# realtimeradio/caltech-bifrost-dsp

Measured on AMD Instinct MI355X. Metric: xengine_ingest_gbps_704in_96ch, higher is better.
Workload: dtype int8 (4+4-bit samples) -> int32

## Files before the change

caltech-bifrost-dsp_amd/csrc/xcorr.hip:

```cpp
#include <algorithm>
#include <cstdlib>
#include <map>
#include <mutex>
#include <vector>

#include "xcorr_kernels.h"
#include "slab.h"
#include "xeng_common.h"

namespace xeng {

struct XgpuConfig {
    int nstand = 352, npol = 2, nchan = 96, ntime_gulp = 480, max_gulps = 0;
};

struct XgpuContext {
    bool live = false;
    int gpu = 0;
    XgpuConfig cfg;
    int ncu = 256;
    int ninput = 0, nblk64 = 0, gkt = 0, cap_kt = 0, cap_gulps = 0, kt_stage = 1;
    int ct_pitch = 0;
    bool raw = false;
    bool kloop16 = false;
    FragGroup* fgroups_dev = nullptr;
    int nfg = 0;
    WorkList work;
    WorkList work_pairs;
    size_t gulp_bytes = 0;
    const uint8_t* gulp_ptr[XC_MAX_GULPS] = {};
    int64_t per_chan = 0, matlen = 0;
    uint8_t* stash[2] = {nullptr, nullptr};
    size_t stash_bytes = 0;
    int cur = 0;
    WgDesc* descs_dev = nullptr;
    int nwg = 0;
    hipStream_t stream = nullptr;
    static constexpr int NMM = 8;
    hipStream_t stream_mm2[NMM] = {};
    int nmm = 2;
    unsigned long long nlaunch = 0;
    hipStream_t stream_mm = nullptr;
    struct Writer { unsigned long long seq; int stream; };
    std::map<const void*, Writer> writers;
    static constexpr int NEV = 256;
    hipEvent_t ev_ring[NEV] = {};
    const void* ring_buf[NEV][2] = {};
    unsigned long long last_seq[NMM] = {};
    hipEvent_t ev_ct = nullptr;
    unsigned long long staging_seen = ~0ull;
    unsigned long long area_seq[2] = {0, 0};
    unsigned long long dump_seq[4] = {0, 0, 0, 0};
    unsigned long long ndump = 0;
    int nfilled = 0;
    bool acc_started = false;
    void* acc_out = nullptr;
    uint8_t* in_dev = nullptr;
    int32_t* out_dev = nullptr;
    unsigned long long* stamps = nullptr;
    GulpDesc* gdesc_dev[2] = {nullptr, nullptr};
    SlabArgs* gargs_dev[2] = {nullptr, nullptr};
    SlabSite slab_site;
    SlabIndexSite slab_index;
    SlabIndexJob slab_job;
    int slab_forced = 0;
    int slab_hint_seen = 0;
    int slab_recent_irr[8] = {}, slab_recent_n[8] = {}, slab_recent_pos = 0;
    unsigned long long slab_tables_until = 0;
    int slab_force_tables = -1;
    bool slab_mode = false;
    EventTimer timer;
};

static std::mutex g_mu;
static XgpuConfig g_cfg;
static XgpuContext g_ctx;
static unsigned long long g_epoch = 1;
// ... 264 lines not shown
    XgpuContext& x = g_ctx;
    if (!x.live || !buf) return 0;
    auto it = x.writers.find(buf);
    return it == x.writers.end() ? 0 : it->second.seq;
}

int xgpu_launches_poll(unsigned long long upto, unsigned long long ctx, bool* done, hipEvent_t* ev, bool exact) {
    std::lock_guard<std::mutex> lk(g_mu);
    XgpuContext& x = g_ctx;
    *done = true;
    if (ev) *ev = nullptr;
    if (upto == 0 || !x.live || ctx != g_ctx_gen) return XENG_STATUS_SUCCESS;
    for (int k = 0; k < (exact ? 1 : x.nmm) && (unsigned long long)k < upto; k++) {
        if (hipEvent_t e = launch_event(upto - k)) {
            const hipError_t q = hipEventQuery(e);
            if (q == hipErrorNotReady) {
                (void)hipGetLastError();
                *done = false;
                if (ev && !*ev) *ev = e;
            } else if (q != hipSuccess) {
                XENG_HIP(q);
            }
        }
    }
    return XENG_STATUS_SUCCESS;
}

int xgpu_pending_poll(unsigned long long seq, unsigned long long epoch, bool* done, bool* launched, hipEvent_t* ev, int* gpu) {
    std::lock_guard<std::mutex> lk(g_mu);
    XgpuContext& x = g_ctx;
    *done = true;
    *launched = true;
    if (ev) *ev = nullptr;
    if (seq == 0 || !x.live || epoch != g_epoch) return XENG_STATUS_SUCCESS;
    if (x.nlaunch < seq) {
        *done = false;
        *launched = false;
        return XENG_STATUS_SUCCESS;
    }
    if (hipEvent_t e = launch_event(seq)) {
        const hipError_t q = hipEventQuery(e);
        if (q == hipErrorNotReady) {
            (void)hipGetLastError();
            *done = false;
            if (ev) *ev = e;
            if (gpu) *gpu = x.gpu;
        } else if (q != hipSuccess) {
            XENG_HIP(q);
        }
    }
    return XENG_STATUS_SUCCESS;
}

}

using namespace xeng;

extern "C" {

int xengXgpuConfigure(int nstand, int npol, int nchan, int ntime_gulp, int max_gulps_per_flush) {
    if (npol != 2) XENG_FAIL(XENG_STATUS_UNSUPPORTED, "xgpu: npol must be 2 (got %d)", npol);
    if (nstand <= 0 || nstand % 4) XENG_FAIL(XENG_STATUS_INVALID_ARGUMENT, "xgpu: nstand must be a positive multiple of 4 (got %d)", nstand);
    if (nstand * npol > 255 * 64) XENG_FAIL(XENG_STATUS_UNSUPPORTED, "xgpu: too many inputs (%d)", nstand * npol);
    if (nchan <= 0 || ntime_gulp <= 0 || max_gulps_per_flush < 0)
        XENG_FAIL(XENG_STATUS_INVALID_ARGUMENT, "xgpu: bad sizes nchan=%d ntime_gulp=%d max_gulps=%d", nchan, ntime_gulp, max_gulps_per_flush);
    std::lock_guard<std::mutex> lk(g_mu);
    g_cfg.nstand = nstand; g_cfg.npol = npol; g_cfg.nchan = nchan; g_cfg.ntime_gulp = ntime_gulp;
    g_cfg.max_gulps = max_gulps_per_flush;
    return XENG_STATUS_SUCCESS;
}

static int initialize_locked(int gpu);

int xengXgpuInitialize(int gpu) {
    std::lock_guard<std::mutex> lk(g_mu);
    destroy_locked();
    const int rc = initialize_locked(gpu);
    if (rc) destroy_locked();
    return rc;
}

static int initialize_locked(int gpu) {
    XgpuContext& x = g_ctx;
    x.cfg = g_cfg;
    x.gpu = gpu < 0 ? 0 : gpu;
    XENG_HIP(hipSetDevice(x.gpu));
    {
        int ncu = 0;
        XENG_HIP(hipDeviceGetAttribute(&ncu, hipDeviceAttributeMultiprocessorCount, x.gpu));
        const char* e = diag_env("XENG_GRID");
        x.ncu = e ? atoi(e) : ncu;
        if (x.ncu < 1) x.ncu = 1;
    }
    x.ninput = x.cfg.nstand * x.cfg.npol;
    x.nblk64 = (x.ninput + 63) / 64;
    x.gkt = (x.cfg.ntime_gulp + 31) / 32;
    x.kt_stage = XC_KT;
    int cap = x.cfg.max_gulps > 0 ? x.cfg.max_gulps : std::max(1, 4800 / (x.gkt * 32));
    cap = std::min(cap, std::max(1, 65535 / (x.gkt * 32)));
    {
        const char* r = getenv("XENG_RAW");
        x.gulp_bytes = (size_t)x.cfg.ntime_gulp * x.cfg.nchan * x.ninput;
        x.raw = !(r && !strcmp(r, "0")) && x.ninput % 16 == 0 &&
                x.cfg.ntime_gulp % (XC_KT * 32) == 0 && x.gulp_bytes + (size_t)16 * x.cfg.nchan * x.ninput < (1ull << 32) &&
                (size_t)x.cfg.nchan * x.ninput >= 128;
        if (x.raw) cap = std::min(cap, XC_MAX_GULPS);
        const char* kl = getenv("XENG_KLOOP");
        x.kloop16 = x.raw && kl && !strcmp(kl, "16");
        const char* st = getenv("XENG_SLAB_TABLES");
        x.slab_force_tables = st ? (strcmp(st, "0") ? 1 : 0) : -1;
        x.slab_hint_seen = 0; x.slab_recent_pos = 0; x.slab_tables_until = 0;
        for (int k = 0; k < 8; k++) x.slab_recent_irr[k] = x.slab_recent_n[k] = 0;
    }
    x.cap_gulps = cap;
    x.cap_kt = ((cap * x.gkt + x.kt_stage - 1) / x.kt_stage) * x.kt_stage;
    x.per_chan = (int64_t)(x.cfg.nstand / 2 + 1) * (x.cfg.nstand / 4) * x.cfg.npol * x.cfg.npol * 4;
    x.matlen = x.per_chan * x.cfg.nchan;
    x.stash_bytes = (size_t)x.cfg.nchan * x.nblk64 * x.cap_kt * KT_BYTES;
    if (x.ninput % 16 == 0) {
        int pitch = x.ninput;
        while (((pitch / 4) & 63) != 8) pitch += 16;
        if ((size_t)16 * pitch + 1024 <= 64 * 1024) x.ct_pitch = pitch;
    }
    if (x.raw) x.stash_bytes = (size_t)cap * x.gulp_bytes;

    for (int b = 0; b < 2; b++) {
        XENG_HIP(hipMalloc((void**)&x.stash[b], x.stash_bytes));
        XENG_HIP(hip_memset_now(x.stash[b], 0, x.stash_bytes));
    }
    XENG_HIP(hipEventCreateWithFlags(&x.ev_ct, hipEventDisableTiming));
    if (x.raw) {
        for (int b = 0; b < 2; b++) {
            XENG_HIP(hipMalloc((void**)&x.gdesc_dev[b], XC_MAX_GULPS * sizeof(GulpDesc)));
            XENG_HIP(hip_memset_now(x.gdesc_dev[b], 0, XC_MAX_GULPS * sizeof(GulpDesc)));
            XENG_HIP(hipMalloc((void**)&x.gargs_dev[b], XC_MAX_GULPS * sizeof(SlabArgs)));
            XENG_HIP(hip_memset_now(x.gargs_dev[b], 0, XC_MAX_GULPS * sizeof(SlabArgs)));
        }
        if (int rcs = slab_site_create(&x.slab_site)) return rcs;
    }
    std::vector<WgDesc> descs = build_wg_descs(x.nblk64);
    x.nwg = (int)descs.size();
    if (x.raw) {
        const bool tiles64 = getenv("XENG_TILING") && !strcmp(getenv("XENG_TILING"), "64");
        const bool plain_order = diag_env("XENG_ITEM_ORDER") && !strcmp(diag_env("XENG_ITEM_ORDER"), "plain");
        const std::vector<FragGroup> groups = tiles64 ? frag_groups_from_tiles(x.nblk64) : build_frag_groups(x.nblk64);
        if (check_frag_groups(groups, x.nblk64) != -1) XENG_FAIL(XENG_STATUS_DEVICE_ERROR, "xgpu: the tiling of %d blocks is not an exact cover", x.nblk64);
        x.nfg = (int)groups.size();
        XENG_HIP(hipMalloc((void**)&x.fgroups_dev, groups.size() * sizeof(FragGroup)));
        XENG_HIP(hipMemcpy(x.fgroups_dev, groups.data(), groups.size() * sizeof(FragGroup), hipMemcpyHostToDevice));
        const std::vector<uint64_t> masks = group_block_masks(groups);
        x.work = build_work(fused_grid(x.cfg.nchan, x.nfg, x.ncu), x.cfg.nchan, x.nfg, plain_order ? nullptr : &masks);
        XENG_HIP(hipMalloc((void**)&x.work.dev, x.work.entries.size() * sizeof(WorkEntry)));
        XENG_HIP(hipMemcpy(x.work.dev, x.work.entries.data(), x.work.entries.size() * sizeof(WorkEntry), hipMemcpyHostToDevice));
        x.work_pairs = build_work(fused_grid(x.cfg.nchan, x.nfg, x.ncu), x.cfg.nchan, x.nfg, plain_order ? nullptr : &masks, true);
        XENG_HIP(hipMalloc((void**)&x.work_pairs.dev, x.work_pairs.entries.size() * sizeof(WorkEntry)));
        XENG_HIP(hipMemcpy(x.work_pairs.dev, x.work_pairs.entries.data(), x.work_pairs.entries.size() * sizeof(WorkEntry), hipMemcpyHostToDevice));
    }
    XENG_HIP(hipMalloc((void**)&x.descs_dev, descs.size() * sizeof(WgDesc)));
    XENG_HIP(hipMemcpy(x.descs_dev, descs.data(), descs.size() * sizeof(WgDesc), hipMemcpyHostToDevice));
    if (const char* o = diag_env("XENG_STREAM_ORDER")) {
        hipStream_t tmp;
        for (const char* c = o; *c; c++) {
            const StreamId id = *c == 'c' ? STREAM_COPY : *c == 'm' ? STREAM_MAP : *c == 'b' ? STREAM_BEAM : *c == 'k' ? STREAM_CONSUMER : STREAM_XGPU;
            int rc0 = get_stream(id, &tmp);
            if (rc0) return rc0;
        }
    }
    int rc = get_stream(STREAM_XGPU, &x.stream);
    if (rc) return rc;
    if (const char* e = diag_env("XENG_MM_STREAMS")) x.nmm = std::max(1, std::min(XgpuContext::NMM, atoi(e)));
    for (int t = 0; t < x.nmm; t++) {
        rc = get_stream(mm_stream_id(t), &x.stream_mm2[t]);
        if (rc) return rc;
    }
    for (int k = 0; k < XgpuContext::NEV; k++) XENG_HIP(hipEventCreateWithFlags(&x.ev_ring[k], hipEventDisableTiming));
    x.stream_mm = x.stream_mm2[0];
    if (diag_env("XENG_DBG_STAMPS")) {
        const int ng = std::max(x.nwg, x.nfg);
        XENG_HIP(hipMalloc((void**)&x.stamps, (size_t)x.cfg.nchan * ng * 4 * 8 * sizeof(unsigned long long)));
        XENG_HIP(hip_memset_now(x.stamps, 0, (size_t)x.cfg.nchan * ng * 4 * 8 * sizeof(unsigned long long)));
    }
    XENG_HIP(hipStreamSynchronize(nullptr));
    x.live = true;
    return XENG_STATUS_SUCCESS;
}

int xengXgpuDestroy(void) {
    std::lock_guard<std::mutex> lk(g_mu);
    return destroy_locked();
}

static void drain_timer() {
    std::lock_guard<std::mutex> lk(g_mu);
    if (g_ctx.live) g_ctx.timer.drain();
}

static int wait_for_event_slot(bool may_block = true) {
    for (;;) {
        hipEvent_t ev = nullptr;
        int gpu = 0;
        {
            std::lock_guard<std::mutex> lk(g_mu);
            XgpuContext& x = g_ctx;
            if (!x.live) return XENG_STATUS_SUCCESS;
            const unsigned long long next = x.nlaunch + 1;
            if (next <= (unsigned long long)XgpuContext::NEV) return XENG_STATUS_SUCCESS;
            ev = x.ev_ring[next % XgpuContext::NEV];
            gpu = x.gpu;
            if (hipEventQuery(ev) == hipSuccess) return XENG_STATUS_SUCCESS;
            (void)hipGetLastError();
        }
        if (!may_block) XENG_FAIL(XENG_STATUS_WOULD_BLOCK, "xgpu: %d launches in flight (xengXgpuWaitLaunchSlot, then retry)", XgpuContext::NEV);
        XENG_HIP(hipSetDevice(gpu));
        XENG_HIP(hipEventSynchronize(ev));
    }
}

int xengXgpuKernel(const void* in_dev, void* out_dev, int doDump) {
    PendingWait pw;
    int rc0 = wait_for_event_slot();
    if (rc0) return rc0;
    {
        std::lock_guard<std::mutex> lk(g_mu);
        int rc = kernel_locked(in_dev, out_dev, doDump, true, &pw);
        if (rc) return rc;
    }
    int rc = wait_unlocked(pw);
    if (rc) return rc;
    if (doDump) drain_timer();
    return XENG_STATUS_SUCCESS;
}

int xengXgpuKernelAsync(const void* in_dev, void* out_dev, int doDump) {
    int rc0 = wait_for_event_slot();
    if (rc0) return rc0;
    std::lock_guard<std::mutex> lk(g_mu);
// ... 306 lines not shown
        const hipError_t re = hipEventRecord(ev, s);
        if (re != hipSuccess) { give_event(ev); XENG_HIP(re); }
    }
    return finish_consumer(ev);
}

int xengXgpuReorder(const void* in_host, void* out_host, const int32_t* bl, const int32_t* conj) {
    XgpuConfig cfg;
    {
        std::lock_guard<std::mutex> lk(g_mu);
        cfg = g_ctx.live ? g_ctx.cfg : g_cfg;
    }
    if (!in_host || !out_host || !bl || !conj) XENG_FAIL(XENG_STATUS_INVALID_ARGUMENT, "Reorder: null buffer");
    const int64_t per_chan = (int64_t)(cfg.nstand / 2 + 1) * (cfg.nstand / 4) * cfg.npol * cfg.npol * 4;
    const int64_t matlen = per_chan * cfg.nchan;
    const size_t nbl = (size_t)cfg.nstand * cfg.nstand * cfg.npol * cfg.npol;
    const long bad = reorder_host((const int32_t*)in_host, (int32_t*)out_host, bl, conj, nbl, cfg.nchan, per_chan, matlen);
    if (bad >= 0) XENG_FAIL(XENG_STATUS_INVALID_ARGUMENT, "Reorder: baseline index %d out of range", bl[bad]);
    return XENG_STATUS_SUCCESS;
}

int xengXgpuGetInfo(int* nstand, int* npol, int* nchan, int* ntime_gulp, int64_t* matlen, int* max_gulps) {
    std::lock_guard<std::mutex> lk(g_mu);
    XgpuContext& x = g_ctx;
    if (!x.live) XENG_FAIL(XENG_STATUS_INVALID_STATE, "xgpu: not initialized");
    if (nstand) *nstand = x.cfg.nstand;
    if (npol) *npol = x.cfg.npol;
    if (nchan) *nchan = x.cfg.nchan;
    if (ntime_gulp) *ntime_gulp = x.cfg.ntime_gulp;
    if (matlen) *matlen = x.matlen;
    if (max_gulps) *max_gulps = x.cap_gulps;
    return XENG_STATUS_SUCCESS;
}

int xengXgpuGetPath(int* fused_corner_turn, int* fp6) {
    std::lock_guard<std::mutex> lk(g_mu);
    XgpuContext& x = g_ctx;
    if (!x.live) XENG_FAIL(XENG_STATUS_INVALID_STATE, "xgpu: not initialized");
    if (fused_corner_turn) *fused_corner_turn = x.raw ? 1 : 0;
    if (fp6) *fp6 = 0;
    return XENG_STATUS_SUCCESS;
}

int xengXgpuGetKernel(int* waves_per_group, int* mfma_k) {
    std::lock_guard<std::mutex> lk(g_mu);
    XgpuContext& x = g_ctx;
    if (!x.live) XENG_FAIL(XENG_STATUS_INVALID_STATE, "xgpu: not initialized");
    const bool k16 = x.raw && x.kloop16;
    if (waves_per_group) *waves_per_group = k16 ? 8 : 4;
    if (mfma_k) *mfma_k = k16 ? 64 : 32;
    return XENG_STATUS_SUCCESS;
}

int xengXgpuSetProfiling(int enable) {
    std::lock_guard<std::mutex> lk(g_mu);
    g_ctx.timer.enabled = enable != 0;
    return XENG_STATUS_SUCCESS;
}

int xengXgpuGetTimes(double ms[2], int count[2]) {
    std::lock_guard<std::mutex> lk(g_mu);
    XgpuContext& x = g_ctx;
    if (x.live && x.stream) {
        XENG_HIP(hipStreamSynchronize(x.stream));
        for (int t = 0; t < x.nmm; t++) XENG_HIP(hipStreamSynchronize(x.stream_mm2[t]));
        x.timer.drain();
    }
    for (int k = 0; k < 2; k++) {
        if (ms) ms[k] = x.timer.total_ms[k];
        if (count) count[k] = x.timer.count[k];
        x.timer.total_ms[k] = 0;
        x.timer.count[k] = 0;
    }
    return XENG_STATUS_SUCCESS;
}

int xengXgpuDebugReadStamps(unsigned long long* host, size_t nwords, int* nwaves) {
    std::lock_guard<std::mutex> lk(g_mu);
    XgpuContext& x = g_ctx;
    if (!x.live || !x.stamps) XENG_FAIL(XENG_STATUS_INVALID_STATE, "stamps not enabled");
    const int ng = x.raw ? x.nfg : x.nwg;
    const size_t n = (size_t)x.cfg.nchan * ng * 4 * 8;
    if (nwaves) *nwaves = x.cfg.nchan * ng * 4;
    for (int t = 0; t < x.nmm; t++) XENG_HIP(hipStreamSynchronize(x.stream_mm2[t]));
    if (host) XENG_HIP(hipMemcpy(host, x.stamps, std::min(nwords, n) * sizeof(unsigned long long), hipMemcpyDeviceToHost));
    return XENG_STATUS_SUCCESS;
}

int xengXgpuDebugReadStash(void* host, size_t nbytes, int* cap_kt, int* nblk64) {
    std::lock_guard<std::mutex> lk(g_mu);
    XgpuContext& x = g_ctx;
    if (!x.live) XENG_FAIL(XENG_STATUS_INVALID_STATE, "xgpu: not initialized");
    if (cap_kt) *cap_kt = x.cap_kt;
    if (nblk64) *nblk64 = x.nblk64;
    if (host) {
        XENG_HIP(hipStreamSynchronize(x.stream));
        XENG_HIP(hipMemcpy(host, x.stash[x.cur], std::min(nbytes, x.stash_bytes), hipMemcpyDeviceToHost));
    }
    return XENG_STATUS_SUCCESS;
}

}
```

caltech-bifrost-dsp_amd/ffi.py:

```python
import ctypes
import os

import numpy as np

_HERE = os.path.dirname(os.path.abspath(__file__))
LIB_PATH = os.environ.get("XENG_LIB") or os.path.join(_HERE, "libxeng.so")

STATUS_SUCCESS = 0
SPACE_SYSTEM, SPACE_CUDA, SPACE_CUDA_HOST = 1, 2, 3

_lib = None


class XengError(RuntimeError):
    def __init__(self, fn, status, msg):
        super().__init__("%s returned %d: %s" % (fn, status, msg))
        self.status = status


class XENGarray(ctypes.Structure):
    _fields_ = [("data", ctypes.c_void_p), ("space", ctypes.c_int), ("dtype", ctypes.c_int),
                ("ndim", ctypes.c_int), ("shape", ctypes.c_long * 8), ("strides", ctypes.c_long * 8),
                ("immutable", ctypes.c_int), ("big_endian", ctypes.c_int), ("conjugated", ctypes.c_int)]


class XengStamp(ctypes.Structure):
    _fields_ = [("w", ctypes.c_ulonglong * 16)]


STATUS_WOULD_BLOCK, STATUS_END_OF_DATA = 6, 7
STREAMS = {"xgpu": 1, "map": 2, "beam": 4, "copy": 8, "consumer": 16, "xgpu_out": 32}
STAMP_NOW_FN = ctypes.CFUNCTYPE(None, ctypes.c_void_p, ctypes.POINTER(ctypes.c_ulonglong))
STAMP_DONE_FN = ctypes.CFUNCTYPE(ctypes.c_int, ctypes.c_void_p, ctypes.POINTER(ctypes.c_ulonglong))
STAMP_WAIT_FN = ctypes.CFUNCTYPE(None, ctypes.c_void_p, ctypes.POINTER(ctypes.c_ulonglong))

_vp, _i, _sz = ctypes.c_void_p, ctypes.c_int, ctypes.c_size_t
_pi = ctypes.POINTER(ctypes.c_int)
_pa = ctypes.POINTER(XENGarray)
_ll, _pll, _psz, _pvp = ctypes.c_longlong, ctypes.POINTER(ctypes.c_longlong), ctypes.POINTER(ctypes.c_size_t), ctypes.POINTER(ctypes.c_void_p)
_pst = ctypes.POINTER(XengStamp)
SYMBOLS = {
    "xengStampNow": [_pst], "xengStampNowFor": [_pst, _vp, ctypes.c_uint], "xengStampDone": [_pst, _pi, _pi], "xengStampWait": [_pst],
    "xengRingCreate": [_pvp, ctypes.c_char_p, _i], "xengRingDestroy": [_vp], "xengRingResize": [_vp, _sz, _sz], "xengRingSetRecycle": [_vp, _i], "xengRingDeclareStreams": [_vp, ctypes.c_uint], "xengRingGetStampClasses": [_vp, ctypes.POINTER(ctypes.c_uint), ctypes.POINTER(ctypes.c_uint), ctypes.POINTER(ctypes.c_uint)],
    "xengRingGetInfo": [_vp, _psz, _psz, _psz, _pi, _pll, ctypes.POINTER(ctypes.c_ulonglong)],
    "xengRingBeginSequence": [_vp, _ll, ctypes.c_char_p, _sz, _i, _pll], "xengRingEndSequence": [_vp, _ll], "xengRingEndWriting": [_vp],
    "xengRingReserve": [_vp, _ll, _sz, _i, _i, _pvp, _pll], "xengRingCommit": [_vp, _ll, _ll, _sz],
    "xengRingCommitExternal": [_vp, _ll, _vp, _sz, _i],
    "xengRingOpenReader": [_vp, _i, _pi], "xengRingCloseReader": [_vp, _i],
    "xengRingNextSequence": [_vp, _i, _i, _pll, _pll, _pi, _pvp, _psz],
    "xengRingAcquire": [_vp, _i, _sz, _sz, _i, _pvp, _psz, _pll, _psz], "xengRingSpanRelease": [_ll],
    "xengRingAcquireParts": [_vp, _i, _sz, _sz, _i, _pvp, _psz, _pll, _pi, _psz],
    "xengRingSetStampHooks": [_vp, STAMP_NOW_FN, STAMP_DONE_FN, STAMP_WAIT_FN, _vp],
    "xengGetDeviceCount": [_pi], "xengSetDevice": [_i], "xengGetDevice": [_pi], "xengDeviceSynchronize": [],
    "xengGetDeviceInfo": [_i, _pi, _pi, ctypes.POINTER(_sz), ctypes.c_char_p, _i], "xengGetDevicePciBusId": [_i, ctypes.c_char_p, _i],
    "xengMalloc": [ctypes.POINTER(_vp), _sz, _i], "xengFree": [_vp, _i], "xengMemcpy": [_vp, _vp, _sz],
    "xengMemcpyAsync": [_vp, _vp, _sz], "xengMemset": [_vp, _i, _sz], "xengStreamSynchronize": [],
    "xengXgpuConfigure": [_i, _i, _i, _i, _i], "xengXgpuInitialize": [_i], "xengXgpuDestroy": [],
    "xengXgpuKernel": [_vp, _vp, _i], "xengXgpuKernelAsync": [_vp, _vp, _i], "xengXgpuKernelAsyncAcc": [_vp, _vp, _i, _vp, _i], "xengXgpuTryKernelAsyncAcc": [_vp, _vp, _i, _vp, _i], "xengXgpuWaitLaunchSlot": [],
    "xengXgpuKernelAsyncSlab": [_vp, _i, _sz, ctypes.c_uint64, _i, _vp, _i, _vp, _i], "xengXgpuTryKernelAsyncSlab": [_vp, _i, _sz, ctypes.c_uint64, _i, _vp, _i, _vp, _i], "xengXgpuGetSlabFallbacks": [_pi], "xengXgpuGetSlabStats": [_pi, _pi], "xengXgpuSync": [], "xengXgpuSyncLag": [_i], "xengXgpuDumpDone": [_i, _pi], "xengXgpuReset": [],
    "xengXgpuCorrelate": [_vp, _vp, _i], "xengXgpuGetOrder": [_vp, _vp, _vp],
    "xengXgpuSubSelect": [_vp, _vp, _vp, _vp, _i, _i], "xengXgpuReorder": [_vp, _vp, _vp, _vp],
    "xengXgpuGetInfo": [_pi, _pi, _pi, _pi, ctypes.POINTER(ctypes.c_int64), _pi],
    "xengXgpuGetPath": [_pi, _pi], "xengXgpuGetKernel": [_pi, _pi],
    "xengXgpuPacketize": [_vp, _vp, _vp, _vp, _i],
    "xengSnap2Unpack": [_vp, _i, ctypes.c_size_t, _vp, ctypes.c_uint64, _i, _i, _i, _i, _i, _pi, _pi],
    "xengSnap2UnpackAsync": [_vp, _i, ctypes.c_size_t, _vp, ctypes.c_uint64, _i, _i, _i, _i, _i],
    "xengSnap2GetAsyncDrops": [_pi], "xengSnap2StampSeq": [_vp, _i, _sz, ctypes.c_uint64, _i],
    "xengXgpuSetProfiling": [_i], "xengXgpuGetTimes": [ctypes.POINTER(ctypes.c_double), _pi],
    "xengMapAssignI32": [_vp, _vp, _sz], "xengMapAddI32": [_vp, _vp, _sz], "xengMapSync": [],
    "xengMapSumI32": [_vp, _pvp, _i, _sz, _i],
    "xengBeamformInitialize": [_i, _i, _i, _i, _i, _i], "xengBeamformDestroy": [],
    "xengBeamformRun": [_vp, _vp, _vp], "xengBeamformRunVersioned": [_vp, _vp, _vp, ctypes.c_longlong], "xengBeamformTryRunVersioned": [_vp, _vp, _vp, ctypes.c_longlong],
    "xengBeamformRunParts": [_vp, _i, _vp, _vp, _vp, ctypes.c_longlong], "xengBeamformTryRunParts": [_vp, _i, _vp, _vp, _vp, ctypes.c_longlong],
    "xengBeamformRunSlabs": [_vp, _i, _i, _vp, _i, _sz, ctypes.c_uint64, _i, _vp, _vp, ctypes.c_longlong], "xengBeamformTryRunSlabs": [_vp, _i, _i, _vp, _i, _sz, ctypes.c_uint64, _i, _vp, _vp, ctypes.c_longlong], "xengBeamformGetSlabFallbacks": [_pi], "xengBeamformGetSlabStats": [_pi, _pi],
    "xengBeamformIntegrate": [_vp, _vp, _i],
    "xengBeamformIntegrateSingleBeam": [_vp, _vp, _i, _i], "xengBeamformMark": [ctypes.POINTER(ctypes.c_ulonglong)], "xengBeamformWait": [ctypes.c_ulonglong], "xengBeamformTicketDone": [ctypes.c_ulonglong, _pi], "xengBeamformSync": [],
    "xengBeamformPacketizeVoltages": [_vp, _vp, _i, _i, _i, _i, _i, _sz, _i, _i, _i, _i, _i, ctypes.c_uint64],
    "xengBeamformSetProfiling": [_i], "xengBeamformGetTimes": [ctypes.POINTER(ctypes.c_double), _pi],
    "xengBeamformGetRouteInfo": [_pi, _pi, _pi],
    "xengUpchanInitialize": [_i, _i, _i, _i, _i, _i, _i], "xengUpchanInitializeDualPol": [_i, _i, _i, _i, _i, _i, _i], "xengUpchanRun": [_vp, _vp, _vp, _ll], "xengUpchanRunParts": [_vp, _i, _vp, _vp, _vp, _ll],
    "xengUpchanMark": [ctypes.POINTER(ctypes.c_ulonglong)], "xengUpchanWait": [ctypes.c_ulonglong], "xengUpchanTicketDone": [ctypes.c_ulonglong, _pi],
    "xengUpchanSync": [], "xengUpchanDestroy": [], "xengUpchanSetPfb": [_i, ctypes.POINTER(ctypes.c_float)], "xengUpchanReset": [],
    "xengUpchanCorrInitialize": [_i, _i, _i, _i, _i, _i, _i, _i], "xengUpchanCorrGetInfo": [_pi, _pi],
    "xengUpchanCorrAccumulate": [_vp], "xengUpchanCorrAccumulateParts": [_vp, _i, _vp], "xengUpchanCorrDump": [_vp], "xengUpchanCorrReset": [],
    "xengUpchanCorrMark": [ctypes.POINTER(ctypes.c_ulonglong)], "xengUpchanCorrWait": [ctypes.c_ulonglong], "xengUpchanCorrTicketDone": [ctypes.c_ulonglong, _pi],
    "xengUpchanCorrSync": [], "xengUpchanCorrDestroy": [], "xengUpchanCorrSetPfb": [_i, ctypes.POINTER(ctypes.c_float)],
    "xengUpchanCorrPrime": [_vp], "xengUpchanCorrPrimeParts": [_vp, _i, _vp],
    "xengUpchanSumBeamsInitialize": [_i, _i, _i, _i, _i, _i, _i, _i], "xengUpchanSumBeamsGetInfo": [_pi, _pi, _pi],
    "xengUpchanSumBeamsRun": [_vp, _vp], "xengUpchanSumBeamsSetPfb": [_i, ctypes.POINTER(ctypes.c_float)], "xengUpchanSumBeamsPrime": [_vp],
    "xengUpchanSumBeamsReset": [], "xengUpchanSumBeamsMark": [ctypes.POINTER(ctypes.c_ulonglong)], "xengUpchanSumBeamsWait": [ctypes.c_ulonglong],
    "xengUpchanSumBeamsTicketDone": [ctypes.c_ulonglong, _pi], "xengUpchanSumBeamsSync": [], "xengUpchanSumBeamsDestroy": [],
    "xengUpchanSpectraInitialize": [_i, _i, _i, _i, _i, _i], "xengUpchanSpectraGetInfo": [_pi, _pi, _pi],
    "xengUpchanSpectraRun": [_vp, _vp], "xengUpchanSpectraRunParts": [_vp, _i, _vp, _vp], "xengUpchanSpectraSetPfb": [_i, ctypes.POINTER(ctypes.c_float)],
    "xengUpchanSpectraPrime": [_vp], "xengUpchanSpectraPrimeParts": [_vp, _i, _vp], "xengUpchanSpectraReset": [],
    "xengUpchanSpectraMark": [ctypes.POINTER(ctypes.c_ulonglong)], "xengUpchanSpectraWait": [ctypes.c_ulonglong],
    "xengUpchanSpectraTicketDone": [ctypes.c_ulonglong, _pi], "xengUpchanSpectraSync": [], "xengUpchanSpectraDestroy": [],
    "xengDedispInitialize": [_i, _i, _i, _i, _i, _i, _i], "xengDedispSetDelays": [_pi], "xengDedispSetWeights": [ctypes.POINTER(ctypes.c_float)],
    "xengDedispRun": [_vp, _i, _vp], "xengDedispReset": [], "xengDedispGetInfo": [_pi, ctypes.POINTER(ctypes.c_longlong)],
    "xengDedispMark": [ctypes.POINTER(ctypes.c_ulonglong)], "xengDedispWait": [ctypes.c_ulonglong], "xengDedispTicketDone": [ctypes.c_ulonglong, _pi],
    "xengDedispSync": [], "xengDedispDestroy": [], "xengDedispCheckGuards": [_pi],
    "xengPulseInitialize": [_i, _i, _i, _i, _i, _i, _i], "xengPulseRun": [_vp, _i, _vp], "xengPulseReset": [],
    "xengPulseGetInfo": [ctypes.POINTER(ctypes.c_longlong), ctypes.POINTER(ctypes.c_longlong)],
    "xengPulseGetBaseline": [ctypes.POINTER(ctypes.c_float), ctypes.POINTER(ctypes.c_float), ctypes.POINTER(ctypes.c_float)],
    "xengPulseCheckGuards": [_pi], "xengPulseMark": [ctypes.POINTER(ctypes.c_ulonglong)], "xengPulseWait": [ctypes.c_ulonglong],
    "xengPulseTicketDone": [ctypes.c_ulonglong, _pi], "xengPulseSync": [], "xengPulseDestroy": [],
    "xengFoldInitialize": [_i, _i, _i, _i, _i, _i],
    "xengFoldSetPhase": [ctypes.POINTER(ctypes.c_ulonglong), ctypes.POINTER(ctypes.c_ulonglong), _pll, ctypes.POINTER(ctypes.c_ubyte), _ll],
    "xengFoldSetRotations": [_pi], "xengFoldSetWeights": [ctypes.POINTER(ctypes.c_float)], "xengFoldRun": [_vp, _i],
    "xengFoldDump": [_vp, ctypes.POINTER(ctypes.c_uint), _i, _i, _i], "xengFoldReset": [], "xengFoldGetInfo": [_pll, _pll],
    "xengFoldCheckGuards": [_pi], "xengFoldMark": [ctypes.POINTER(ctypes.c_ulonglong)], "xengFoldWait": [ctypes.c_ulonglong],
    "xengFoldTicketDone": [ctypes.c_ulonglong, _pi], "xengFoldSync": [], "xengFoldDestroy": [],
    "xengPeriodInitialize": [_i, _i, _i, _i, _i, _i, _i, _i, _i, _i], "xengPeriodSetMask": [ctypes.POINTER(ctypes.c_ubyte)],
    "xengPeriodRun": [_vp, _i, _vp, _pi], "xengPeriodReset": [], "xengPeriodGetInfo": [_pll, _pi, _pll],
    "xengPeriodGetSpectrum": [ctypes.POINTER(ctypes.c_float), _pi], "xengPeriodCheckGuards": [_pi],
    "xengPeriodMark": [ctypes.POINTER(ctypes.c_ulonglong)], "xengPeriodWait": [ctypes.c_ulonglong],
    "xengPeriodTicketDone": [ctypes.c_ulonglong, _pi], "xengPeriodSync": [], "xengPeriodDestroy": [],
# ... 153 lines not shown
```

include/xeng.h:

```cpp
#ifndef XENG_H_
#define XENG_H_

#include <stddef.h>
#include <stdint.h>

#ifdef __cplusplus
extern "C" {
#endif

#define XENG_STATUS_SUCCESS            0
#define XENG_STATUS_INVALID_ARGUMENT   1
#define XENG_STATUS_INVALID_STATE      2
#define XENG_STATUS_DEVICE_ERROR       3
#define XENG_STATUS_UNSUPPORTED        4
#define XENG_STATUS_MEM_ALLOC_FAILED   5
#define XENG_STATUS_WOULD_BLOCK        6
#define XENG_STATUS_END_OF_DATA        7

#define XENG_SPACE_AUTO       0
#define XENG_SPACE_SYSTEM     1
#define XENG_SPACE_CUDA       2
#define XENG_SPACE_CUDA_HOST  3

#define XENG_MAX_DIMS 8
// ... 57 lines not shown
int xengRingCloseReader(xengRing *ring, int reader);
int xengRingNextSequence(xengRing *ring, int reader, int may_block, long long *seq, long long *time_tag, int *nringlet,
                         const void **header, size_t *header_len);
int xengRingAcquire(xengRing *ring, int reader, size_t advance, size_t gulp_nbytes, int may_block, void **data, size_t *nbytes,
                    long long *span, size_t *skipped);
int xengRingAcquireParts(xengRing *ring, int reader, size_t advance, size_t gulp_nbytes, int may_block, void *data[2], size_t nbytes[2],
                         long long span[2], int *nparts, size_t *skipped);
int xengRingSpanRelease(long long span);
typedef void (*xengRingStampNowFn)(void *user, unsigned long long stamp[2]);
typedef int (*xengRingStampDoneFn)(void *user, const unsigned long long stamp[2]);
typedef void (*xengRingStampWaitFn)(void *user, const unsigned long long stamp[2]);
int xengRingSetStampHooks(xengRing *ring, xengRingStampNowFn now, xengRingStampDoneFn done, xengRingStampWaitFn wait, void *user);


int xengXgpuConfigure(int nstand, int npol, int nchan, int ntime_gulp, int max_gulps_per_flush);

int xengXgpuInitialize(int gpu);
int xengXgpuDestroy(void);

int xengXgpuKernel(const void *in_dev, void *out_dev, int doDump);

int xengXgpuKernelAsync(const void *in_dev, void *out_dev, int doDump);
int xengXgpuKernelAsyncAcc(const void *in_dev, void *out_dev, int doDump, void *acc_dev, int acc_mode);
int xengXgpuTryKernelAsyncAcc(const void *in_dev, void *out_dev, int doDump, void *acc_dev, int acc_mode);
int xengXgpuWaitLaunchSlot(void);
int xengXgpuKernelAsyncSlab(const void *packets_dev, int npkt, size_t pkt_stride, uint64_t seq0, int chan0_pipeline, void *out_dev,
                            int doDump, void *acc_dev, int acc_mode);
int xengXgpuTryKernelAsyncSlab(const void *packets_dev, int npkt, size_t pkt_stride, uint64_t seq0, int chan0_pipeline, void *out_dev,
                               int doDump, void *acc_dev, int acc_mode);
int xengXgpuGetSlabFallbacks(int *nfallback);
int xengXgpuGetSlabStats(int *nscattered, int *nirregular);
int xengXgpuSync(void);
int xengXgpuSyncLag(int lag);
int xengXgpuDumpDone(int lag, int *done);

int xengXgpuReset(void);

int xengXgpuCorrelate(const void *in_host, void *out_host, int doDump);

int xengXgpuGetOrder(const int32_t *antpol_to_input, int32_t *antpol_to_bl, int32_t *is_conj);

int xengXgpuSubSelect(const void *in_dev, void *out_dev, const int32_t *vismap_dev,
                      const int32_t *conj_dev, int nvis, int nchan_sum);

int xengXgpuPacketize(const void *in_dev, void *out_dev, const int32_t *antpol_to_bl_dev,
                      const int32_t *is_conj_dev, int fmt);

int xengXgpuReorder(const void *in_host, void *out_host, const int32_t *antpol_to_bl, const int32_t *is_conj);

int xengXgpuGetInfo(int *nstand, int *npol, int *nchan, int *ntime_gulp, int64_t *matlen, int *max_gulps);

int xengXgpuGetPath(int *fused_corner_turn, int *fp6);
int xengXgpuGetKernel(int *waves_per_group, int *mfma_k);

int xengXgpuSetProfiling(int enable);
int xengXgpuGetTimes(double ms[2], int count[2]);

int xengSnap2Unpack(const void *packets_dev, int npkt, size_t pkt_stride, void *out_dev, uint64_t seq0, int ntime,
                    int chan0_pipeline, int nchan_tot, int npol_tot, int clear, int *nplaced, int *ndropped);
int xengSnap2UnpackAsync(const void *packets_dev, int npkt, size_t pkt_stride, void *out_dev, uint64_t seq0, int ntime,
                         int chan0_pipeline, int nchan_tot, int npol_tot, int clear);
int xengSnap2GetAsyncDrops(int *ndropped);

int xengSnap2StampSeq(void *packets_dev, int npkt, size_t pkt_stride, uint64_t seq0, int pkts_per_seq);

int xengMapAssignI32(void *a_dev, const void *b_dev, size_t nwords);
int xengMapAddI32(void *a_dev, const void *b_dev, size_t nwords);
#define XENG_MAP_SUM_MAX 16
int xengMapSumI32(void *a_dev, const void *const *srcs_dev, int nsrc, size_t nwords, int add);
int xengMapSync(void);


int xengBeamformInitialize(int gpu, int ninput, int nchan, int ntime, int nbeam, int ntime_blocks);
int xengBeamformDestroy(void);

int xengBeamformRun(const void *in_dev, void *out_dev, const void *weights_dev);
int xengBeamformRunVersioned(const void *in_dev, void *out_dev, const void *weights_dev, long long weights_version);
int xengBeamformTryRunVersioned(const void *in_dev, void *out_dev, const void *weights_dev, long long weights_version);
int xengBeamformRunParts(const void *in0_dev, int ntime0, const void *in1_dev, void *out_dev, const void *weights_dev, long long weights_version);
int xengBeamformTryRunParts(const void *in0_dev, int ntime0, const void *in1_dev, void *out_dev, const void *weights_dev, long long weights_version);
int xengBeamformRunSlabs(const void *packets0_dev, int npkt0, int ntime0, const void *packets1_dev, int npkt1, size_t pkt_stride,
                         uint64_t seq0, int chan0_pipeline, void *out_dev, const void *weights_dev, long long weights_version);
int xengBeamformTryRunSlabs(const void *packets0_dev, int npkt0, int ntime0, const void *packets1_dev, int npkt1, size_t pkt_stride,
                            uint64_t seq0, int chan0_pipeline, void *out_dev, const void *weights_dev, long long weights_version);
int xengBeamformGetSlabFallbacks(int *nfallback);
int xengBeamformGetSlabStats(int *nscattered, int *nirregular);

int xengBeamformIntegrate(const void *in_dev, void *out_dev, int ntime_sum);

int xengBeamformIntegrateSingleBeam(const void *in_dev, void *out_dev, int ntime_sum, int beam_id);
int xengBeamformPacketizeVoltages(const void *in_dev, void *out_dev, int nchan, int nbeam, int ntime, int beam0, int nbeam_pkt,
                                  size_t pkt_stride, int server, int gbe, int nbeam_hdr, int nserver, int chan0, uint64_t seq0);
int xengBeamformSync(void);
int xengBeamformMark(unsigned long long *ticket);
int xengBeamformWait(unsigned long long ticket);
int xengBeamformTicketDone(unsigned long long ticket, int *done);
int xengBeamformSetProfiling(int enable);
int xengBeamformGetTimes(double ms[2], int count[2]);
int xengBeamformGetRouteInfo(int *tiles_total, int *tiles_bf16, int *outlier_inputs);

int xengUpchanInitialize(int gpu, int ninput, int nchan, int ntime, int nupchan, int nbeam, int nframe_sum);
int xengUpchanInitializeDualPol(int gpu, int ninput, int nchan, int ntime, int nupchan, int nbeam, int nframe_sum);
int xengUpchanRun(const void *in_dev, void *out_dev, const void *weights_dev, long long weights_version);
int xengUpchanRunParts(const void *in0_dev, int ntime0, const void *in1_dev, void *out_dev, const void *weights_dev,
                       long long weights_version);
int xengUpchanSetPfb(int ntap, const float *coeffs);
// ... 181 lines not shown
```

Baseline: 5992.

## Autotune the k-loop kernel variant with an init-time timing probe

```diff
diff --git a/caltech-bifrost-dsp_amd/csrc/xcorr.hip b/caltech-bifrost-dsp_amd/csrc/xcorr.hip
--- a/caltech-bifrost-dsp_amd/csrc/xcorr.hip
+++ b/caltech-bifrost-dsp_amd/csrc/xcorr.hip
@@ -1,10 +1,12 @@
 #include <algorithm>
+#include <chrono>
 #include <cstdlib>
 #include <map>
 #include <mutex>
 #include <vector>
 
 #include "xcorr_kernels.h"
+#include "xcorr_choice.h"
 #include "slab.h"
 #include "xeng_common.h"
 
@@ -23,6 +25,10 @@
     int ct_pitch = 0;
     bool raw = false;
     bool kloop16 = false;
+    int choice_source = XENG_KERNEL_CHOICE_DEFAULT;
+    int probe_blocks[KERNEL_CHOICE_MAX_CAND] = {};
+    double probe_median_ms[KERNEL_CHOICE_MAX_CAND] = {};
+    double probe_cost_ms = 0;
     FragGroup* fgroups_dev = nullptr;
     int nfg = 0;
     WorkList work;
@@ -393,6 +399,114 @@
     return XENG_STATUS_SUCCESS;
 }
 
+
+__global__ void probe_fill_kernel(uint32_t* dst, size_t nwords) {
+    for (size_t i = blockIdx.x * (size_t)blockDim.x + threadIdx.x; i < nwords; i += (size_t)gridDim.x * blockDim.x) {
+        uint32_t h = (uint32_t)i * 0x9E3779B1u + 0x7F4A7C15u;
+        h ^= h >> 16; h *= 0x85EBCA6Bu; h ^= h >> 13; h *= 0xC2B2AE35u; h ^= h >> 16;
+        dst[i] = h;
+    }
+}
+
+static_assert(XENG_KERNEL_CHOICE_MAX_CANDIDATES == KERNEL_CHOICE_MAX_CAND, "xeng.h and xcorr_choice.h disagree");
+constexpr int PROBE_BLOCKS = 4;
+constexpr int PROBE_LEAD = 4;
+constexpr int PROBE_TIMED = 28;
+
+static bool probe_eligible(const XgpuContext& x) {
+    return x.raw && (int64_t)x.cfg.nchan * x.nfg >= x.ncu;
+}
+
+static int reset_launch_state_locked() {
+    XgpuContext& x = g_ctx;
+    for (int k = 0; k < XgpuContext::NEV; k++) {
+        if (x.ev_ring[k]) XENG_HIP(hipEventDestroy(x.ev_ring[k]));
+        x.ev_ring[k] = nullptr;
+        XENG_HIP(hipEventCreateWithFlags(&x.ev_ring[k], hipEventDisableTiming));
+        x.ring_buf[k][0] = x.ring_buf[k][1] = nullptr;
+    }
+    x.nlaunch = 0;
+    x.writers.clear();
+    for (int t = 0; t < XgpuContext::NMM; t++) x.last_seq[t] = 0;
+    x.staging_seen = ~0ull;
+    x.area_seq[0] = x.area_seq[1] = 0;
+    for (int k = 0; k < 4; k++) x.dump_seq[k] = 0;
+    x.ndump = 0;
+    x.cur = 0;
+    x.nfilled = 0;
+    x.acc_started = false;
+    x.acc_out = nullptr;
+    x.slab_mode = false;
+    for (int g = 0; g < XC_MAX_GULPS; g++) x.gulp_ptr[g] = nullptr;
+    return XENG_STATUS_SUCCESS;
+}
+
+static int probe_kernels_locked() {
+    XgpuContext& x = g_ctx;
+    const auto t0 = std::chrono::steady_clock::now();
+    const size_t in_bytes = (size_t)x.cap_gulps * x.gulp_bytes;
+    const size_t out_bytes = (size_t)x.matlen * 2 * sizeof(int32_t);
+    uint8_t* in = nullptr;
+    int32_t* out[2] = {nullptr, nullptr};
+    hipEvent_t ev[2] = {nullptr, nullptr};
+    bool have = hipMalloc((void**)&in, in_bytes) == hipSuccess && hipMalloc((void**)&out[0], out_bytes) == hipSuccess &&
+                hipMalloc((void**)&out[1], out_bytes) == hipSuccess && hipEventCreate(&ev[0]) == hipSuccess && hipEventCreate(&ev[1]) == hipSuccess;
+    constexpr int NCAND = 2;
+    const bool cand_k16[NCAND] = {false, true};
+    std::vector<double> times[NCAND];
+    auto run = [&]() -> int {
+        const size_t nwords = in_bytes / 4;
+        const unsigned blocks = (unsigned)std::min<size_t>(4096, (nwords + 255) / 256);
+        hipLaunchKernelGGL(probe_fill_kernel, dim3(blocks), dim3(256), 0, x.stream_mm, (uint32_t*)in, nwords);
+        XENG_HIP(hipGetLastError());
+        XENG_HIP(hipStreamSynchronize(x.stream_mm));
+        unsigned long long n = 0;
+        for (int b = 0; b < NCAND * PROBE_BLOCKS; b++) {
+            const int c = b % NCAND;
+            x.kloop16 = cand_k16[c];
+            for (int i = 0; i < PROBE_LEAD + PROBE_TIMED; i++, n++) {
+                for (int g = 0; g < x.cap_gulps; g++)
+                    if (int rc = kernel_locked(in + (size_t)g * x.gulp_bytes, out[n & 1], g == x.cap_gulps - 1, false, nullptr)) return rc;
+                const hipStream_t s = x.stream_mm2[(x.nlaunch - 1) % x.nmm];
+                if (i == PROBE_LEAD - 1) XENG_HIP(hipEventRecord(ev[0], s));
+                if (i == PROBE_LEAD + PROBE_TIMED - 1) XENG_HIP(hipEventRecord(ev[1], s));
+                if (x.ndump >= 2)
+                    if (hipEvent_t e = launch_event(x.dump_seq[(x.ndump - 2) & 3])) XENG_HIP(hipEventSynchronize(e));
+            }
+            for (int t = 0; t < x.nmm; t++) XENG_HIP(hipStreamSynchronize(x.stream_mm2[t]));
+            float ms = 0;
+            XENG_HIP(hipEventElapsedTime(&ms, ev[0], ev[1]));
+            times[c].push_back((double)ms / PROBE_TIMED);
+        }
+        return XENG_STATUS_SUCCESS;
+    };
+    int rc = have ? run() : XENG_STATUS_SUCCESS;
+    if (!have) (void)hipGetLastError();
+    if (x.stream) (void)hipStreamSynchronize(x.stream);
+    for (int t = 0; t < x.nmm; t++) (void)hipStreamSynchronize(x.stream_mm2[t]);
+    for (hipEvent_t e : ev) if (e) (void)hipEventDestroy(e);
+    if (in) (void)hipFree(in);
+    for (int32_t* o : out) if (o) (void)hipFree(o);
+    x.kloop16 = false;
+    if (rc) return rc;
+    rc = reset_launch_state_locked();
+    if (rc) return rc;
+    if (have) {
+        const double* blk[NCAND];
+        int nblk[NCAND];
+        for (int c = 0; c < NCAND; c++) {
+            blk[c] = times[c].data();
+            nblk[c] = (int)times[c].size();
+            x.probe_blocks[c] = nblk[c];
+            x.probe_median_ms[c] = block_stats(blk[c], nblk[c]).median;
+        }
+        x.kloop16 = cand_k16[choose_kernel_candidate(blk, nblk, NCAND)];
+        x.choice_source = XENG_KERNEL_CHOICE_PROBE;
+    }
+    x.probe_cost_ms = std::chrono::duration<double, std::milli>(std::chrono::steady_clock::now() - t0).count();
+    return XENG_STATUS_SUCCESS;
+}
+
 }
 
 using namespace xeng;
@@ -447,7 +561,10 @@
                 (size_t)x.cfg.nchan * x.ninput >= 128;
         if (x.raw) cap = std::min(cap, XC_MAX_GULPS);
         const char* kl = getenv("XENG_KLOOP");
+        const char* kp = getenv("XENG_KLOOP_PROBE");
         x.kloop16 = x.raw && kl && !strcmp(kl, "16");
+        if (kl && (!strcmp(kl, "16") || !strcmp(kl, "32"))) x.choice_source = XENG_KERNEL_CHOICE_FORCED;
+        else if (kp && !strcmp(kp, "0")) x.choice_source = XENG_KERNEL_CHOICE_PROBE_OFF;
         const char* st = getenv("XENG_SLAB_TABLES");
         x.slab_force_tables = st ? (strcmp(st, "0") ? 1 : 0) : -1;
         x.slab_hint_seen = 0; x.slab_recent_pos = 0; x.slab_tables_until = 0;
@@ -523,6 +640,8 @@
     }
     XENG_HIP(hipStreamSynchronize(nullptr));
     x.live = true;
+    if (x.choice_source == XENG_KERNEL_CHOICE_DEFAULT && probe_eligible(x))
+        if (int rcp = probe_kernels_locked()) return rcp;
     return XENG_STATUS_SUCCESS;
 }
 
@@ -935,6 +1054,26 @@
     return XENG_STATUS_SUCCESS;
 }
 
+int xengXgpuGetKernelChoice(int* waves_per_group, int* contraction_streams, int* decided_by, int* ncandidates, int* cand_waves,
+                            int* cand_streams, double* cand_median_ms, int* cand_blocks, double* probe_ms) {
+    std::lock_guard<std::mutex> lk(g_mu);
+    XgpuContext& x = g_ctx;
+    if (!x.live) XENG_FAIL(XENG_STATUS_INVALID_STATE, "xgpu: not initialized");
+    if (waves_per_group) *waves_per_group = x.raw && x.kloop16 ? 8 : 4;
+    if (contraction_streams) *contraction_streams = x.nmm;
+    if (decided_by) *decided_by = x.choice_source;
+    const int nc = x.choice_source == XENG_KERNEL_CHOICE_PROBE ? 2 : 0;
+    if (ncandidates) *ncandidates = nc;
+    for (int c = 0; c < XENG_KERNEL_CHOICE_MAX_CANDIDATES; c++) {
+        if (cand_waves) cand_waves[c] = c < nc ? (c == 0 ? 4 : 8) : 0;
+        if (cand_streams) cand_streams[c] = c < nc ? x.nmm : 0;
+        if (cand_median_ms) cand_median_ms[c] = c < nc ? x.probe_median_ms[c] : 0.0;
+        if (cand_blocks) cand_blocks[c] = c < nc ? x.probe_blocks[c] : 0;
+    }
+    if (probe_ms) *probe_ms = x.probe_cost_ms;
+    return XENG_STATUS_SUCCESS;
+}
+
 int xengXgpuSetProfiling(int enable) {
     std::lock_guard<std::mutex> lk(g_mu);
     g_ctx.timer.enabled = enable != 0;
diff --git a/caltech-bifrost-dsp_amd/csrc/xcorr_choice.h b/caltech-bifrost-dsp_amd/csrc/xcorr_choice.h
--- /dev/null
+++ b/caltech-bifrost-dsp_amd/csrc/xcorr_choice.h
@@ -0,0 +1,46 @@
+#pragma once
+#include <algorithm>
+#include <cmath>
+#include <vector>
+
+namespace xeng {
+
+constexpr int KERNEL_CHOICE_MIN_BLOCKS = 4;
+constexpr int KERNEL_CHOICE_MAX_CAND = 4;
+
+struct BlockStats {
+    bool ok = false;
+    double lo = 0, hi = 0, median = 0;
+};
+
+inline BlockStats block_stats(const double* ms, int n) {
+    BlockStats s;
+    if (!ms || n < KERNEL_CHOICE_MIN_BLOCKS) return s;
+    std::vector<double> v(ms, ms + n);
+    for (double t : v)
+        if (!std::isfinite(t) || t <= 0) return s;
+    std::sort(v.begin(), v.end());
+    s.lo = v.front();
+    s.hi = v.back();
+    s.median = n % 2 ? v[n / 2] : 0.5 * (v[n / 2 - 1] + v[n / 2]);
+    s.ok = true;
+    return s;
+}
+
+inline int choose_kernel_candidate(const double* const* blocks, const int* nblocks, int ncand) {
+    if (!blocks || !nblocks || ncand < 2) return 0;
+    const BlockStats d = block_stats(blocks[0], nblocks[0]);
+    if (!d.ok) return 0;
+    int best = 0;
+    double best_median = d.median;
+    for (int c = 1; c < ncand; c++) {
+        const BlockStats s = block_stats(blocks[c], nblocks[c]);
+        if (!s.ok) continue;
+        if (!(s.hi < d.lo)) continue;
+        if (!(d.median - s.median > d.hi - d.lo)) continue;
+        if (s.median < best_median) { best = c; best_median = s.median; }
+    }
+    return best;
+}
+
+}
diff --git a/caltech-bifrost-dsp_amd/ffi.py b/caltech-bifrost-dsp_amd/ffi.py
--- a/caltech-bifrost-dsp_amd/ffi.py
+++ b/caltech-bifrost-dsp_amd/ffi.py
@@ -62,6 +62,7 @@
     "xengXgpuSubSelect": [_vp, _vp, _vp, _vp, _i, _i], "xengXgpuReorder": [_vp, _vp, _vp, _vp],
     "xengXgpuGetInfo": [_pi, _pi, _pi, _pi, ctypes.POINTER(ctypes.c_int64), _pi],
     "xengXgpuGetPath": [_pi, _pi], "xengXgpuGetKernel": [_pi, _pi],
+    "xengXgpuGetKernelChoice": [_pi, _pi, _pi, _pi, _pi, _pi, ctypes.POINTER(ctypes.c_double), _pi, ctypes.POINTER(ctypes.c_double)],
     "xengXgpuPacketize": [_vp, _vp, _vp, _vp, _i],
     "xengSnap2Unpack": [_vp, _i, ctypes.c_size_t, _vp, ctypes.c_uint64, _i, _i, _i, _i, _i, _pi, _pi],
     "xengSnap2UnpackAsync": [_vp, _i, ctypes.c_size_t, _vp, ctypes.c_uint64, _i, _i, _i, _i, _i],
diff --git a/include/xeng.h b/include/xeng.h
--- a/include/xeng.h
+++ b/include/xeng.h
@@ -133,6 +133,13 @@
 
 int xengXgpuGetPath(int *fused_corner_turn, int *fp6);
 int xengXgpuGetKernel(int *waves_per_group, int *mfma_k);
+#define XENG_KERNEL_CHOICE_DEFAULT 0
+#define XENG_KERNEL_CHOICE_PROBE 1
+#define XENG_KERNEL_CHOICE_FORCED 2
+#define XENG_KERNEL_CHOICE_PROBE_OFF 3
+#define XENG_KERNEL_CHOICE_MAX_CANDIDATES 4
+int xengXgpuGetKernelChoice(int *waves_per_group, int *contraction_streams, int *decided_by, int *ncandidates, int *cand_waves,
+                            int *cand_streams, double *cand_median_ms, int *cand_blocks, double *probe_ms);
 
 int xengXgpuSetProfiling(int enable);
 int xengXgpuGetTimes(double ms[2], int count[2]);
diff --git a/profiles/kernel_choice_report.py b/profiles/kernel_choice_report.py
--- /dev/null
+++ b/profiles/kernel_choice_report.py
@@ -0,0 +1,43 @@
+#!/usr/bin/env python3
+import argparse
+import ctypes
+import json
+import os
+import sys
+import time
+
+ROOT = os.path.dirname(os.path.dirname(os.path.abspath(__file__)))
+sys.path.insert(0, ROOT)
+
+
+def main():
+    ap = argparse.ArgumentParser()
+    ap.add_argument("--rounds", type=int, default=5)
+    ap.add_argument("--shape", default="352,96,480,5", help="nstand,nchan,ntime_gulp,gulps per integration")
+    args = ap.parse_args()
+    import caltech_bifrost_dsp_amd
+    from caltech_bifrost_dsp_amd import ffi
+    nstand, nchan, ntime, gps = (int(v) for v in args.shape.split(","))
+    ffi.call("xengSetDevice", 0)
+    for rnd in range(args.rounds):
+        for probe in ("0", None):
+            if probe is None:
+                os.environ.pop("XENG_KLOOP_PROBE", None)
+            else:
+                os.environ["XENG_KLOOP_PROBE"] = probe
+            ffi.call("xengXgpuConfigure", nstand, 2, nchan, ntime, gps)
+            t0 = time.perf_counter()
+            ffi.call("xengXgpuInitialize", 0)
+            init_ms = (time.perf_counter() - t0) * 1e3
+            w, s, by, nc, ms = ctypes.c_int(), ctypes.c_int(), ctypes.c_int(), ctypes.c_int(), ctypes.c_double()
+            cw, cs, cb, cm = (ctypes.c_int * 4)(), (ctypes.c_int * 4)(), (ctypes.c_int * 4)(), (ctypes.c_double * 4)()
+            ffi.call("xengXgpuGetKernelChoice", ctypes.byref(w), ctypes.byref(s), ctypes.byref(by), ctypes.byref(nc), cw, cs, cm, cb, ctypes.byref(ms))
+            ffi.call("xengXgpuDestroy")
+            print(json.dumps({"round": rnd, "XENG_KLOOP_PROBE": probe, "initialize_ms": round(init_ms, 2), "waves": w.value, "streams": s.value,
+                              "decided_by": by.value, "probe_ms": round(ms.value, 2),
+                              "candidates": [{"waves": cw[i], "streams": cs[i], "median_ms": round(cm[i], 5), "blocks": cb[i]} for i in range(nc.value)]}), flush=True)
+    os.environ.pop("XENG_KLOOP_PROBE", None)
+
+
+if __name__ == "__main__":
+    main()
```

Result: no change. 6030, median of 2 (+0.6%).
